# qiqiqicheng/news-recommendation-tc

Measured on AMD Instinct MI355X. Metric: recalled pairs/sec (YouTubeDNN top-30) + DIN scored pairs/sec, 1/2/4/8 MI355X, higher is better.
Workload: dtype fp16

## Files before the change

### news-recommendation-tc_amd/csrc/ip_topk.hip

```cpp
#include "nrk_common.h"

#include <float.h>
#include <math.h>
#include <stdlib.h>

#include <algorithm>
#include <type_traits>
#include <utility>

namespace nrk {

typedef float f32x16 __attribute__((ext_vector_type(16)));
typedef _Float16 f16x8 __attribute__((ext_vector_type(8)));
typedef unsigned u32x4 __attribute__((ext_vector_type(4)));
typedef float f32x4 __attribute__((ext_vector_type(4)));

constexpr int IP_KFAST = 128;
constexpr int IP_KMAX = 2048;
#ifndef NRK_SCAN_TILE
#define NRK_SCAN_TILE 8192
#endif
constexpr int SCAN_TILE = NRK_SCAN_TILE;
#ifndef NRK_SCAN_TB128
#define NRK_SCAN_TB128 4
// ... 30 lines not shown
static inline size_t catalog_body_bytes(int64_t n_items, int dp) {
    return (size_t)n_blocks_of(n_items) * 64u * (size_t)dp;
}
__host__ __device__ static inline bool catalog_has_hb(int dp) { return dp <= 64; }
__host__ __device__ static inline size_t catalog_hb_offset(int64_t n_items, int dp) {
    return (size_t)n_blocks_of(n_items) * 64u * (size_t)dp + CATALOG_HDR;
}

__global__ void catalog_pack_kernel(const float* __restrict__ items, int64_t n_items, int dim,
                                    int dp, const CatalogHdr* __restrict__ hdr,
                                    uint4* __restrict__ out) {
    const int ds = dp / 16;
    const float scale = hdr->scale;
    const int64_t total = n_blocks_of(n_items) * ds * 64;
    for (int64_t t = blockIdx.x * (int64_t)blockDim.x + threadIdx.x; t < total;
         t += (int64_t)gridDim.x * blockDim.x) {
        const int lane = (int)(t & 63);
        const int s = (int)((t >> 6) % ds);
        const int64_t b = (t >> 6) / ds;
        const int64_t item = b * 32 + (lane & 31);
        const int d0 = 16 * s + 8 * (lane >> 5);
        uint16_t v[8];
#pragma unroll
        for (int e = 0; e < 8; ++e) {
            const int d = d0 + e;
            const float f = (item < n_items && d < dim) ? items[item * dim + d] : 0.0f;
            v[e] = __builtin_bit_cast(uint16_t, (_Float16)(f * scale));
        }
        uint4 o;
        o.x = v[0] | ((uint32_t)v[1] << 16);
        o.y = v[2] | ((uint32_t)v[3] << 16);
        o.z = v[4] | ((uint32_t)v[5] << 16);
        o.w = v[6] | ((uint32_t)v[7] << 16);
        out[t] = o;
    }
}

__global__ void catalog_pack_hb_kernel(const float* __restrict__ items, int64_t n_items, int dim,
                                       int dp, const CatalogHdr* __restrict__ hdr,
                                       uint4* __restrict__ out) {
    const int ppr = dp / 8;
    const float scale = hdr->scale;
    const int64_t total = n_blocks_of(n_items) * 2 * 16 * ppr;
    for (int64_t t = blockIdx.x * (int64_t)blockDim.x + threadIdx.x; t < total;
         t += (int64_t)gridDim.x * blockDim.x) {
        const int p = (int)(t % ppr);
        const int r = (int)((t / ppr) & 15);
        const int64_t q = t / ppr / 16;
        const int64_t item = (q >> 1) * 32 + (r & 3) + 8 * (r >> 2) + 4 * (q & 1);
        uint16_t v[8];
#pragma unroll
        for (int e = 0; e < 8; ++e) {
            const int d = 8 * p + e;
            const float f = (item < n_items && d < dim) ? items[item * dim + d] : 0.0f;
            v[e] = __builtin_bit_cast(uint16_t, (_Float16)(f * scale));
        }
        out[t] = make_uint4(v[0] | ((uint32_t)v[1] << 16), v[2] | ((uint32_t)v[3] << 16),
                            v[4] | ((uint32_t)v[5] << 16), v[6] | ((uint32_t)v[7] << 16));
    }
}

__device__ __forceinline__ int cat_lanes(int dim) { return dim <= 16 ? 16 : dim <= 32 ? 32 : 64; }

__global__ void catalog_norm_kernel(const float* __restrict__ items, int64_t n_items, int dim,
                                    CatalogHdr* hdr) {
    const int lane = threadIdx.x & 63, L = cat_lanes(dim), R = WAVE / L, j = lane & (L - 1);
    const int64_t wid = (blockIdx.x * (int64_t)blockDim.x + threadIdx.x) >> 6;
    const int64_t nw = ((int64_t)gridDim.x * blockDim.x) >> 6;
    float m = 0.0f, a = 0.0f;
    for (int64_t r0 = wid * R; r0 < n_items; r0 += nw * R) {
        const int64_t r = r0 + lane / L;
        float s = 0.0f;
        if (r < n_items) {
            const float* row = items + r * dim;
            for (int d = j; d < dim; d += L) {
                const float x = row[d];
                s += x * x;
                a = fmaxf(a, fabsf(x));
            }
        }
        for (int o = L >> 1; o > 0; o >>= 1) s += __shfl_xor(s, o, WAVE);
        if (r < n_items) m = fmaxf(m, sqrtf(s));
    }
#pragma unroll
    for (int o = 32; o > 0; o >>= 1) {
        m = fmaxf(m, __shfl_xor(m, o, WAVE));
        a = fmaxf(a, __shfl_xor(a, o, WAVE));
    }
    if ((threadIdx.x & 63) == 0) {
        atomicMax((unsigned int*)&hdr->max_norm, __float_as_uint(m));
        atomicMax((unsigned int*)&hdr->max_abs, __float_as_uint(a));
    }
}

__global__ void catalog_dnorm_kernel(const float* __restrict__ items, int64_t n_items, int dim,
                                     CatalogHdr* hdr) {
    const float scale = hdr->scale;
    const int lane = threadIdx.x & 63, L = cat_lanes(dim), R = WAVE / L, j = lane & (L - 1);
    const int64_t wid = (blockIdx.x * (int64_t)blockDim.x + threadIdx.x) >> 6;
    const int64_t nw = ((int64_t)gridDim.x * blockDim.x) >> 6;
    double m = 0.0;
    for (int64_t r0 = wid * R; r0 < n_items; r0 += nw * R) {
        const int64_t r = r0 + lane / L;
        double s = 0.0;
        if (r < n_items) {
            const float* row = items + r * dim;
            for (int d = j; d < dim; d += L) {
                const float f = row[d];
                const float x = (float)(_Float16)(f * scale);
                const double e = (double)x / (double)scale - (double)f;
                s += e * e;
            }
        }
        for (int o = L >> 1; o > 0; o >>= 1) s += __shfl_xor(s, o, WAVE);
        if (r < n_items) m = fmax(m, sqrt(s));
    }
#pragma unroll
    for (int o = 32; o > 0; o >>= 1) m = fmax(m, __shfl_xor(m, o, WAVE));
    if ((threadIdx.x & 63) == 0) atomicMax((unsigned int*)&hdr->max_dnorm, __float_as_uint((float)(m * (1.0 + 1e-6))));
}

__global__ void catalog_hdr_kernel(CatalogHdr* hdr, int dim, int dp) {
    hdr->dim = dim;
    hdr->dp = dp;
    hdr->scale = pow2_scale(hdr->max_abs);
}

__device__ __forceinline__ float round_down_sub(float theta, float two_eps) {
    float c = theta - two_eps;
    return __uint_as_float(c > 0.0f ? __float_as_uint(c) - 1u
                                    : (c == 0.0f ? 0x80000001u : __float_as_uint(c) + 1u));
}

__device__ __forceinline__ uint32_t partner32(uint32_t v, int h) {
    const auto r = __builtin_amdgcn_permlane32_swap(v, v, false, false);
    return h ? (uint32_t)r[0] : (uint32_t)r[1];
}
__device__ __forceinline__ float partner32f(float v, int h) {
    return __uint_as_float(partner32(__float_as_uint(v), h));
}

__device__ __forceinline__ float pair_min32(float v) {
    const auto r = __builtin_amdgcn_permlane32_swap(__float_as_uint(v), __float_as_uint(v), false, false);
    return fminf(__uint_as_float((uint32_t)r[0]), __uint_as_float((uint32_t)r[1]));
}

__device__ __forceinline__ uint32_t add_if(uint32_t x, uint64_t m) {
    uint32_t r;
    uint64_t co;
    asm("v_addc_co_u32_e64 %0, %1, %2, 0, %3" : "=v"(r), "=s"(co) : "v"(x), "s"(m));
    (void)co;
    return r;
}

template <int MT>
__device__ __forceinline__ void top_insert(float (&t)[MT], float v) {
#pragma unroll
    for (int i = MT - 1; i >= 1; --i) t[i] = __builtin_amdgcn_fmed3f(t[i], t[i - 1], v);
    t[0] = fmaxf(t[0], v);
}

#ifndef NRK_SCAN_STAMP
#define NRK_SCAN_STAMP 0
#endif

constexpr int SCAN_PRE_MAX = 64, SCAN_PRE_MIN = 128, SCAN_PRE_DIV = 6, SCAN_SHARD_PRE_DIV = 6;
template <int F, int T>
__device__ __forceinline__ uint32_t sel_mask_c(uint64_t m) {
    uint32_t r;
    asm("v_cndmask_b32_e64 %0, %1, %2, %3" : "=v"(r) : "n"(F), "n"(T), "s"(m));
    return r;
}
template <int T>
__device__ __forceinline__ uint32_t sel_mask_v(uint64_t m, uint32_t f) {
    uint32_t r;
    asm("v_cndmask_b32_e64 %0, %1, %2, %3" : "=v"(r) : "v"(f), "n"(T), "s"(m));
    return r;
}
template <int TB>
__device__ __forceinline__ uint32_t first_set_block(const uint64_t (&am)[TB]) {
    if constexpr (TB == 1) {
        return 0u;
    } else {
        uint32_t bs = sel_mask_c<TB - 1, TB - 2>(am[TB - 2]);
        static_for<TB - 2>([&](auto bc) {
            constexpr int b = TB - 3 - decltype(bc)::value;
            bs = sel_mask_v<b>(am[b], bs);
        });
        return bs;
    }
}
#if NRK_SCAN_STAMP
__device__ unsigned long long scan_stamps[1024 * 16];
#define SC_STAMP(k)                                           \
    do {                                                      \
        const uint64_t t_now_ = __builtin_readcyclecounter(); \
        sstp[k] += t_now_ - t_prev;                           \
        t_prev = t_now_;                                      \
    } while (0)
#else
#define SC_STAMP(k) \
    do {            \
    } while (0)
#endif

template <int MT>
__device__ __forceinline__ void list_bound_out(const float (&t)[MT], bool live, int h, int user, int n_users, int jk,
                                               float* __restrict__ bnd, int bnd_m, const float4* __restrict__ uinfo) {
    const int nl = jk + 1;
    float c[2 * MT];
#pragma unroll
    for (int i = 0; i < MT; ++i) {
        c[i] = t[i];
        c[2 * MT - 1 - i] = partner32f(t[i], h);
    }
#pragma unroll
    for (int d = MT; d >= 1; d >>= 1)
#pragma unroll
        for (int i = 0; i < 2 * MT; ++i)
            if ((i & d) == 0) {
                const float x = c[i], y = c[i + d];
                c[i] = fmaxf(x, y);
                c[i + d] = fminf(x, y);
            }
    if (h == 0 && user < n_users) {
        float* o = bnd + (size_t)user * bnd_m;
        const int p0 = 2 * (MT - nl);
        const float4 ui = uinfo[user];
        const double inv = 1.0 / (double)ui.z;
#pragma unroll
        for (int j = 0; j < 2 * MT; ++j) {
            const int r = j - p0;
            if (r >= 0 && r < bnd_m) {
                float v = -INFINITY;
                if (live && c[j] != -INFINITY) {
                    const double tv = (double)c[j] * inv - (double)ui.w;
                    v = (float)tv;
                    if ((double)v > tv) v = nextafterf(v, -INFINITY);
                }
                o[r] = v;
            }
        }
        for (int r = 2 * nl; r < bnd_m; ++r) o[r] = -INFINITY;
    }
}

template <int DS>
__device__ __forceinline__ void scan_user_setup(const float* __restrict__ users, int n_users, int dim, int user,
                                                int h, float vmax, float dvmax, float sv_scale, f16x8 (&uf)[DS],
                                                float& eps, float& scl, bool& live) {
    constexpr int DP = DS * 16;
    const bool active = user < n_users;
    float uval[DS][8];
    float nrm2 = 0.0f, uabs = 0.0f;
    const float* urow = users + (size_t)(active ? user : 0) * dim;
#pragma unroll
    for (int s = 0; s < DS; ++s)
#pragma unroll
        for (int e = 0; e < 8; ++e) {
            const int d = 16 * s + 8 * h + e;
            const float f = (active && d < dim) ? urow[d] : 0.0f;
            uval[s][e] = f;
            nrm2 += f * f;
            uabs = fmaxf(uabs, fabsf(f));
        }
    nrm2 += __shfl_xor(nrm2, 32, WAVE);
    uabs = fmaxf(uabs, __shfl_xor(uabs, 32, WAVE));
    const float su = pow2_scale(uabs);
    float du2 = 0.0f;
#pragma unroll
    for (int s = 0; s < DS; ++s)
#pragma unroll
        for (int e = 0; e < 8; ++e) {
            const float a = uval[s][e] * su;
            uf[s][e] = (_Float16)a;
            const float d = (float)uf[s][e] - a;
            du2 += d * d;
        }
    du2 += __shfl_xor(du2, 32, WAVE);
    const float nu = sqrtf(nrm2), ndu = sqrtf(du2) / su;
    const float ceps = 3.0517578e-5f + (float)DP * 1.1920929e-7f;
    eps = (nrm2 == 0.0f) ? 0.0f : (ndu * vmax + nu * dvmax + ndu * dvmax + ceps * nu * vmax) * 1.0001f + 1e-30f;
    scl = su * sv_scale;
    live = active && nrm2 > 0.0f;
}

template <int DP, int NW, int NSL, int UG, int MT, int WPE>
__global__ __launch_bounds__(NW * 64, WPE) void ip_scan_kernel(
    const float* __restrict__ users, int n_users, const uint8_t* __restrict__ catalog, int n_items, int dim, int k,
    int m2, uint2* __restrict__ app, int32_t* __restrict__ acnt, float4* __restrict__ uinfo, int tile_lo,
    int tile_hi, int n_pre, int pstride, float* __restrict__ bnd, int bnd_m) {
    constexpr int DS = DP / 16;
    constexpr int BLOCK_BYTES = 64 * DP;
    constexpr int TB = scan_tb(DP);
    constexpr int TILE_BYTES = TB * BLOCK_BYTES;
    constexpr int LPT = TILE_BYTES / (NW * 1024);
    static_assert(LPT >= 1 && LPT * NW * 1024 == TILE_BYTES, "tile split");
    static_assert(NSL >= 2, "ring");
    __shared__ __attribute__((aligned(16))) uint8_t smem[NSL * TILE_BYTES];

    const int tid = threadIdx.x;
    const int wave = tid >> 6, lane = tid & 63, h = lane >> 5, q = lane & 31;
    const int ub = blockIdx.x;
    const int ubase = ub * (NW * 32 * UG) + wave * (32 * UG);
#if NRK_SCAN_STAMP
    uint64_t sstp[8] = {0, 0, 0, 0, 0, 0, 0, 0};
    uint64_t t_prev = 0;
#endif

    const int nblk = (n_items + 31) >> 5;
    const int ntile = tile_hi;
    const CatalogHdr* hdr = reinterpret_cast<const CatalogHdr*>(catalog + (size_t)nblk * BLOCK_BYTES);
    const float vmax = hdr->max_norm, sv_scale = hdr->scale, dvmax = hdr->max_dnorm;
    const int jk = (k + 1) / 2 - 1;

    f16x8 ufrag[UG][DS];
    float eps_s[UG], tau[UG];
    float t[UG][MT];
    bool live[UG];
#pragma unroll
    for (int g = 0; g < UG; ++g) {
        const int user = ubase + g * 32 + q;
        float eps, scl;
        scan_user_setup<DS>(users, n_users, dim, user, h, vmax, dvmax, sv_scale, ufrag[g], eps, scl, live[g]);
        eps_s[g] = eps * scl;
        if (h == 0 && user < n_users) uinfo[user] = make_float4(-INFINITY, eps_s[g], scl, eps);
        tau[g] = live[g] ? -FLT_MAX : INFINITY;
#pragma unroll
        for (int i = 0; i < MT; ++i) t[g][i] = (live[g] && i >= MT - 1 - jk) ? -INFINITY : INFINITY;
    }
    uint2* const wapp = app + (size_t)(ub * (NW * 32 * UG) + __builtin_amdgcn_readfirstlane(wave) * (32 * UG)) *
                                  2 * (size_t)m2;
    uint32_t pos[UG], lim[UG];
#pragma unroll
    for (int g = 0; g < UG; ++g) {
        pos[g] = (uint32_t)((g * 32 + q) * 2 + h) * (uint32_t)m2;
        lim[g] = pos[g] + (uint32_t)m2 - 1u;
    }
    auto slot = [&](uint32_t x, int g) -> uint32_t { return min(x, lim[g]); };
    auto app_store_if = [&](uint64_t m, uint32_t e, uint2 v) {
        const uint32_t off = e << 3;
        const uint64_t d = ((uint64_t)v.y << 32) | v.x;
        uint64_t sv;
// ... 417 lines not shown
            scan_user_setup<DS>(users, n_users, dim, ubase + g * 32 + q, h, vmax, dvmax, sv_scale, ufrag[g], eps, scl,
                                live);
        }
#if NRK_SCAN_WS_PRIO
        __builtin_amdgcn_s_setprio(NRK_SCAN_WS_PRIO);
#endif
        const uint32_t lds0 = lds_base + lane * 16;
        auto pf_issue = [&](int sl, int b, u32x4 (&af)[DS]) {
            const uint32_t base = lds0 + (uint32_t)(sl * TILE_BYTES + b * DS * 1024);
            asm volatile("ds_read_b128 %0, %2 offset:0\n\tds_read_b128 %1, %2 offset:1024"
                         : "=&v"(af[0]), "=&v"(af[1])
                         : "v"(base)
                         : "memory");
        };
        auto pf_wait_issue = [&](u32x4 (&cur)[DS], int sl, int b, u32x4 (&nxt)[DS]) {
            const uint32_t base = lds0 + (uint32_t)(sl * TILE_BYTES + b * DS * 1024);
            asm volatile("s_waitcnt lgkmcnt(0)\n\tds_read_b128 %0, %4 offset:0\n\tds_read_b128 %1, %4 offset:1024"
                         : "=&v"(nxt[0]), "=&v"(nxt[1]), "+v"(cur[0]), "+v"(cur[1])
                         : "v"(base)
                         : "memory");
        };
        auto pf_wait = [&](u32x4 (&cur)[DS]) {
            asm volatile("s_waitcnt lgkmcnt(0)" : "+v"(cur[0]), "+v"(cur[1])::"memory");
        };
        auto tile = [&](auto nt_c, const int (&tt)[TPS], const int (&sl)[TPS], const uint32_t (&ms)[TPS],
                        auto mask_c) __attribute__((always_inline)) {
            constexpr int NT = decltype(nt_c)::value, NBK = NT * TB;
            constexpr bool MASK = decltype(mask_c)::value;
            float mx[2][UG];
            using P5 = float[5];
            auto red1 = [&](const f32x16& a, int bb, P5& pm) __attribute__((always_inline)) {
                float x[16];
#pragma unroll
                for (int r = 0; r < 16; ++r) {
                    x[r] = a[r];
                    if constexpr (MASK) {
                        const int row = (tt[bb / TB] * TB + bb % TB) * 32 + (r & 3) + 8 * (r >> 2) + 4 * h;
                        if (row >= n_items) x[r] = -INFINITY;
                    }
                }
                auto m3 = [](float p, float s, float u) { return fmaxf(fmaxf(p, s), u); };
                pm[0] = m3(x[0], x[1], x[2]);
                pm[1] = m3(x[3], x[4], x[5]);
                pm[2] = m3(x[6], x[7], x[8]);
                pm[3] = m3(x[9], x[10], x[11]);
                pm[4] = fmaxf(m3(x[12], x[13], x[14]), x[15]);
            };
            auto red2 = [&](const P5& pm, int bb, int gg) __attribute__((always_inline)) {
                mx[bb & 1][gg] = fmaxf(fmaxf(fmaxf(fmaxf(pm[0], pm[1]), pm[2]), pm[3]), pm[4]);
            };
            auto put = [&](int bb) __attribute__((always_inline)) {
                const f32x4 v0 = {mx[bb & 1][0], mx[bb & 1][1], mx[bb & 1][2], mx[bb & 1][3]};
                const f32x4 v1 = {mx[bb & 1][4], mx[bb & 1][5], mx[bb & 1][6], mx[bb & 1][7]};
                asm volatile("ds_write_b128 %0, %1 offset:0\n\tds_write_b128 %0, %2 offset:1024" ::"v"(
                                 ms[bb / TB] + (uint32_t)((bb % TB) * 2048)),
                             "v"(v0), "v"(v1)
                             : "memory");
            };
            auto slb = [&](int bb) { return sl[bb / TB]; };
            constexpr int NSTEP = NBK * UG;
            f32x16 acc[2];
            float pm[2][5];
            u32x4 afp[DS], afb[DS];
            pf_issue(slb(0), 0, afp);
            static_for<NBK>([&](auto bc) {
                constexpr int bb = decltype(bc)::value;
                u32x4 afn[DS];
                if constexpr (bb + 1 < NBK) pf_wait_issue(afp, slb(bb + 1), (bb + 1) % TB, afn);
                else pf_wait(afp);
#pragma unroll
                for (int s = 0; s < DS; ++s) afb[s] = afp[s];
                if constexpr (bb + 1 < NBK) {
#pragma unroll
                    for (int s = 0; s < DS; ++s) afp[s] = afn[s];
                }
                static_for<UG>([&](auto gc) {
                    constexpr int g = decltype(gc)::value, j = bb * UG + g;
                    f32x16& A = acc[j & 1];
                    A = __builtin_amdgcn_mfma_f32_32x32x16_f16(__builtin_bit_cast(f16x8, afb[0]), ufrag[g][0],
                                                               f32x16{}, 0, 0, 0);
                    if constexpr (j >= 2) red2(pm[j & 1], (j - 2) / UG, (j - 2) % UG);
                    if constexpr (!MASK) {
                        __builtin_amdgcn_sched_group_barrier(0x008, 1, 0);
                        if constexpr (j >= 2) __builtin_amdgcn_sched_group_barrier(0x002, 3, 0);
                    }
                    A = __builtin_amdgcn_mfma_f32_32x32x16_f16(__builtin_bit_cast(f16x8, afb[1]), ufrag[g][1], A, 0,
                                                               0, 0);
                    if constexpr (j >= 1) red1(acc[(j - 1) & 1], (j - 1) / UG, pm[(j - 1) & 1]);
                    if constexpr (bb > 0 && g == 2) put(bb - 1);
                    if constexpr (!MASK) {
                        __builtin_amdgcn_sched_group_barrier(0x008, 1, 0);
                        if constexpr (j >= 1) __builtin_amdgcn_sched_group_barrier(0x002, 6, 0);
                        __builtin_amdgcn_sched_barrier(0);
                    }
                });
            });
            red2(pm[(NSTEP - 2) & 1], (NSTEP - 2) / UG, (NSTEP - 2) % UG);
            red1(acc[(NSTEP - 1) & 1], (NSTEP - 1) / UG, pm[(NSTEP - 1) & 1]);
            red2(pm[(NSTEP - 1) & 1], (NSTEP - 1) / UG, (NSTEP - 1) % UG);
            put(NBK - 1);
        };
#pragma unroll
        for (int p = 0; p < DAHEAD; ++p) issue_step(p);
        for (int p = 0; p <= NP; ++p) {
            SC_STAMP(7);
            sync();
            SC_STAMP(0);
            issue_step(p + DAHEAD);
            int tts[TPS], sls[TPS];
            uint32_t mss[TPS];
#pragma unroll
            for (int t = 0; t < TPS; ++t) {
                const int i = min(TPS * p + t, nseq - 1);
                tts[t] = seq(i);
                sls[t] = (TPS * p + t) % NSL;
                mss[t] = mx_base + (uint32_t)(((p & 1) * TPS + t) * MXS);
            }
            if (TPS * p + TPS <= nseq) {
                bool full = true;
#pragma unroll
                for (int t = 0; t < TPS; ++t) full = full && tts[t] < full_tiles;
                if (full) tile(std::integral_constant<int, TPS>{}, tts, sls, mss, std::false_type{});
                else tile(std::integral_constant<int, TPS>{}, tts, sls, mss, std::true_type{});
            } else if (TPS * p < nseq) {
                tile(std::integral_constant<int, 1>{}, tts, sls, mss, std::true_type{});
            }
            SC_STAMP(1);
        }
        asm volatile("s_waitcnt vmcnt(0)" ::: "memory");
#if NRK_SCAN_STAMP
        SC_STAMP(2);
        stamp_out();
#endif
        return;
    }

    const int gb = ((wv - NPW) / NPW) * UGB;
    float eps_s[UGB], tau[UGB];
    float t[UGB][MT];
    bool live[UGB];
#pragma unroll
    for (int g = 0; g < UGB; ++g) {
        f16x8 uf[DS];
        float eps, scl;
        const int user = ubase + (gb + g) * 32 + q;
        scan_user_setup<DS>(users, n_users, dim, user, h, vmax, dvmax, sv_scale, uf, eps, scl, live[g]);
        eps_s[g] = eps * scl;
        if (h == 0 && user < n_users) uinfo[user] = make_float4(-INFINITY, eps_s[g], scl, eps);
        tau[g] = live[g] ? -FLT_MAX : INFINITY;
#pragma unroll
        for (int i = 0; i < MT; ++i) t[g][i] = (live[g] && i >= MT - 1 - jk) ? -INFINITY : INFINITY;
    }
    uint2* const wapp = app + (size_t)(ubase + gb * 32) * 2 * (size_t)m2;
    const uint32_t pos0 = (uint32_t)(q * 2 + h) * (uint32_t)m2;
    const uint32_t gstride = 64u * (uint32_t)m2;
    uint32_t pos[UGB];
#pragma unroll
    for (int g = 0; g < UGB; ++g) pos[g] = pos0 + (uint32_t)g * gstride;
    auto slot = [&](uint32_t x, int g) { return min(x, pos0 + (uint32_t)g * gstride + (uint32_t)m2 - 1u); };
    auto app_store_if = [&](uint64_t m, uint32_t e, uint2 v) {
        const uint32_t off = e << 3;
        const uint64_t d = ((uint64_t)v.y << 32) | v.x;
        uint64_t sv;
        asm volatile(
            "s_and_saveexec_b64 %0, %1\n\t"
            "global_store_dwordx2 %2, %3, %4\n\t"
            "s_mov_b64 exec, %0"
            : "=&s"(sv)
            : "s"(m), "v"(off), "v"(d), "s"(wapp)
            : "memory", "scc");
    };
    auto retau = [&](int g) {
        const float lb = pair_min32(t[g][MT - 1]);
        const float c = lb - 2.0f * eps_s[g];
        const float tv = fmaxf(__builtin_fmaf(fabsf(c), -0x1p-22f, c) - 0x1p-120f, -FLT_MAX);
        tau[g] = live[g] ? tv : INFINITY;
    };
    int next_s = n_pre > 0 ? tile_lo : INT_MAX, left_s = n_pre;
#if NRK_SCAN_STAMP
    t_prev = __builtin_readcyclecounter();
#endif
    const uint32_t mq = mx_base + (uint32_t)(gb / 4) * 1024u;
    f32x4 rr[TPS][TB][UGB / 4];
    auto read_issue = [&](int t, uint32_t a) {
        if constexpr (NB == 2) {
            asm volatile(
                "ds_read_b128 %0, %4 offset:0\n\tds_read_b128 %1, %4 offset:2048\n\t"
                "ds_read_b128 %2, %4 offset:4096\n\tds_read_b128 %3, %4 offset:6144"
                : "=&v"(rr[t][0][0]), "=&v"(rr[t][1][0]), "=&v"(rr[t][2][0]), "=&v"(rr[t][3][0])
                : "v"(a)
                : "memory");
        } else {
            asm volatile(
                "ds_read_b128 %0, %8 offset:0\n\tds_read_b128 %1, %8 offset:1024\n\t"
                "ds_read_b128 %2, %8 offset:2048\n\tds_read_b128 %3, %8 offset:3072\n\t"
                "ds_read_b128 %4, %8 offset:4096\n\tds_read_b128 %5, %8 offset:5120\n\t"
                "ds_read_b128 %6, %8 offset:6144\n\tds_read_b128 %7, %8 offset:7168"
                : "=&v"(rr[t][0][0]), "=&v"(rr[t][0][1]), "=&v"(rr[t][1][0]), "=&v"(rr[t][1][1]),
                  "=&v"(rr[t][2][0]), "=&v"(rr[t][2][1]), "=&v"(rr[t][3][0]), "=&v"(rr[t][3][1])
                : "v"(a)
                : "memory");
        }
    };
    static_assert(TPS <= 2, "read_wait");
    auto read_wait = [&](int t, bool left) {
        constexpr int L1 = TB * (UGB / 4);
        if constexpr (NB == 2) {
            if (left)
                asm volatile("s_waitcnt lgkmcnt(%4)"
                             : "+v"(rr[t][0][0]), "+v"(rr[t][1][0]), "+v"(rr[t][2][0]), "+v"(rr[t][3][0])
                             : "n"(L1)
                             : "memory");
            else
                asm volatile("s_waitcnt lgkmcnt(0)"
                             : "+v"(rr[t][0][0]), "+v"(rr[t][1][0]), "+v"(rr[t][2][0]), "+v"(rr[t][3][0])::"memory");
        } else {
            if (left)
                asm volatile("s_waitcnt lgkmcnt(%8)"
                             : "+v"(rr[t][0][0]), "+v"(rr[t][0][1]), "+v"(rr[t][1][0]), "+v"(rr[t][1][1]),
                               "+v"(rr[t][2][0]), "+v"(rr[t][2][1]), "+v"(rr[t][3][0]), "+v"(rr[t][3][1])
                             : "n"(L1)
                             : "memory");
            else
                asm volatile("s_waitcnt lgkmcnt(0)"
                             : "+v"(rr[t][0][0]), "+v"(rr[t][0][1]), "+v"(rr[t][1][0]), "+v"(rr[t][1][1]),
                               "+v"(rr[t][2][0]), "+v"(rr[t][2][1]), "+v"(rr[t][3][0]), "+v"(rr[t][3][1])::"memory");
        }
    };
    float vtp[UGB];
#pragma unroll
    for (int g = 0; g < UGB; ++g) vtp[g] = -INFINITY;
    for (int p = 0; p <= NP; ++p) {
        SC_STAMP(5);
        sync();
        SC_STAMP(0);
        if (p == 0) continue;
        const int p1 = p - 1;
#pragma unroll
        for (int t = 0; t < TPS; ++t)
            if (TPS * p1 + t < nseq) read_issue(t, mq + (uint32_t)(((p1 & 1) * TPS + t) * MXS));
        static_for<TPS>([&](auto tc) {
        constexpr int T = decltype(tc)::value;
        const int j = TPS * p1 + T;
        if (j >= nseq) return;
        read_wait(T, T + 1 < TPS && j + 1 < nseq);
        const int tt = seq(j);
        const bool pre = j < n_pre;
        if (j == n_pre) {
#pragma unroll
            for (int g = 0; g < UGB; ++g) retau(g);
        }
        bool ins_ok = true;
        if (!pre && tt == next_s) {
            ins_ok = false;
            next_s = --left_s > 0 ? next_s + pstride : INT_MAX;
        }
        const auto& r = rr[T];
        SC_STAMP(1);
#if NRK_SCAN_WS_FLOOR
        if (r[0][0][0] != 12345.0f) return;
#endif
        const uint32_t hb0 = (uint32_t)(tt * TB * 2) + (uint32_t)h;
        static_for<UGB>([&](auto gc) {
            constexpr int g = decltype(gc)::value;
            float mx[TB];
#pragma unroll
            for (int b = 0; b < TB; ++b) mx[b] = r[b][g / 4][g % 4];
            const float vt = fmaxf(fmaxf(mx[0], mx[1]), fmaxf(mx[2], mx[3]));
            if (!pre) {
                uint64_t am[TB], gm = 0, multi = 0;
#pragma unroll
                for (int b = 0; b < TB; ++b) {
                    am[b] = __builtin_amdgcn_ballot_w64(mx[b] >= tau[g]);
                    multi |= gm & am[b];
                    gm |= am[b];
                }
                if (gm) {
                    const uint32_t fid = (first_set_block<TB>(am) << 1) + hb0;
                    const uint32_t p0 = pos[g];
                    app_store_if(gm, slot(p0, g), make_uint2(__float_as_uint(vt), fid));
                    uint32_t p = add_if(p0, gm);
                    if (multi) {
                        p = p0;
#pragma unroll
                        for (int b = 0; b < TB; ++b) {
                            app_store_if(am[b] & multi, slot(p, g), make_uint2(__float_as_uint(mx[b]), hb0 + 2u * b));
                            p = add_if(p, am[b]);
                        }
                    }
                    pos[g] = p;
                }
            }
            SC_STAMP(2);
            if (pre) {
                const bool in = vt > t[g][MT - 1];
                if (__builtin_amdgcn_ballot_w64(in)) top_insert<MT>(t[g], in ? vt : -INFINITY);
            } else {
                const float vi = fmaxf(ins_ok ? vt : -INFINITY, vtp[g]);
                if (T + 1 < TPS || ((j - n_pre) & (insp - 1)) < insp - TPS) {
                    vtp[g] = vi;
                } else {
                    vtp[g] = -INFINITY;
                    const bool in = vi > t[g][MT - 1];
                    if (__builtin_amdgcn_ballot_w64(in)) {
                        top_insert<MT>(t[g], in ? vi : -INFINITY);
                        if (!pre) retau(g);
                    }
                }
            }
            SC_STAMP(4);
        });
        });
    }
    {
#pragma unroll
        for (int g = 0; g < UGB; ++g) {
            const bool in = vtp[g] > t[g][MT - 1];
            top_insert<MT>(t[g], in ? vtp[g] : -INFINITY);
        }
    }
    asm volatile("s_waitcnt vmcnt(0)" ::: "memory");
#if NRK_SCAN_STAMP
    SC_STAMP(3);
    stamp_out();
#endif
#pragma unroll
    for (int g = 0; g < UGB; ++g) {
        const float lb = pair_min32(t[g][MT - 1]);
        const int user = ubase + (gb + g) * 32 + q;
        if (user < n_users) {
            acnt[(size_t)user * 2 + h] = (int)(pos[g] - (pos0 + (uint32_t)g * gstride));
            if (h == 0) reinterpret_cast<float*>(uinfo + user)[0] = live[g] ? lb : -INFINITY;
        }
    }
    if constexpr (MT <= 32) {
        if (bnd != nullptr) {
#pragma unroll
            for (int g = 0; g < UGB; ++g)
                list_bound_out<MT>(t[g], live[g], h, ubase + (gb + g) * 32 + q, n_users, jk, bnd, bnd_m, uinfo);
        }
    }
}

__device__ __forceinline__ uint32_t fkey(float f) {
    const uint32_t b = __float_as_uint(f);
    return (b >> 31) ? ~b : (b | 0x80000000u);
}
__device__ __forceinline__ float fkey_inv(uint32_t k) {
    return __uint_as_float((k >> 31) ? (k & 0x7FFFFFFFu) : ~k);
}

template <int E>
__device__ __forceinline__ void lds_ranks(const uint32_t* __restrict__ row, int c, const uint32_t (&mine)[E],
                                          int pos, int (&rank)[E]) {
#pragma unroll
    for (int e = 0; e < E; ++e) rank[e] = 0;
    for (int j0 = 0; j0 < c; j0 += 4) {
        const uint4 q = *reinterpret_cast<const uint4*>(row + j0);
        const uint32_t qq[4] = {q.x, q.y, q.z, q.w};
#pragma unroll
        for (int t = 0; t < 4; ++t) {
#pragma unroll
            for (int e = 0; e < E; ++e)
                rank[e] += (qq[t] > mine[e] || (qq[t] == mine[e] && j0 + t < e * WAVE + pos)) ? 1 : 0;
        }
    }
}

__device__ __forceinline__ uint32_t wave_sort_desc_u32(uint32_t x, int lane) {
    static_for<6>([&](auto klc) {
        constexpr int kl = decltype(klc)::value + 1, k = 1 << kl;
        static_for<kl>([&](auto jc) {
            constexpr int j = 1 << (kl - 1 - decltype(jc)::value);
            const uint32_t y = lane_xor<j>(x);
            const bool up = (lane & k) == 0;
            const bool lower = (lane & j) == 0;
            x = (lower == up) ? max(x, y) : min(x, y);
        });
    });
    return x;
}

__device__ __forceinline__ uint32_t lds_select(uint32_t* __restrict__ row, int c, int r, int lane) {
    if (c <= WAVE) {
        wave_sync_lds();
        const uint32_t srt = wave_sort_desc_u32(lane < c ? row[lane] : 0u, lane);
        return (uint32_t)__builtin_amdgcn_readlane((int)srt, r);
    }
    if (lane < 4) row[c + lane] = 0u;
    wave_sync_lds();
    uint32_t x = 0u;
    for (int b0 = 0; b0 < c; b0 += WAVE) {
        const uint32_t mine[1] = {b0 + lane < c ? row[b0 + lane] : 0u};
        int rank[1];
        lds_ranks<1>(row, c, mine, b0 + lane, rank);
        const unsigned long long b = __ballot(b0 + lane < c && rank[0] == r);
        if (b) {
            x = (uint32_t)__shfl((int)mine[0], __ffsll((long long)b) - 1, WAVE);
            break;
        }
    }
    return x;
}

#ifndef NRK_SH_WG
#define NRK_SH_WG 6
#endif
constexpr int SH_WG_PER_CU = NRK_SH_WG;
constexpr int SH_ENT = 4;

__device__ __forceinline__ void sh_load(const uint2* s0, const uint2* s1, int a0, int n, int b0, int lane,
                                        uint2 (&ent)[SH_ENT]) {
#pragma unroll
    for (int j = 0; j < SH_ENT; ++j) {
        const int e = b0 + j * WAVE + lane;
        ent[j] = e < n ? (e < a0 ? s0[e] : s1[e - a0]) : make_uint2(0u, 0u);
    }
}

__global__ __launch_bounds__(256) void ip_select_kernel(
    int64_t n_users, int k, int m2, int bandcap, const uint2* __restrict__ app,
    const int32_t* __restrict__ acnt, const float4* __restrict__ uinfo, uint2* __restrict__ cand,
    int32_t* __restrict__ cand_cnt, float2* __restrict__ ucut, int32_t* __restrict__ ovf_flag,
    int32_t* __restrict__ ovf_list, int32_t* __restrict__ ovf_count) {
    __shared__ __attribute__((aligned(16))) uint32_t sel[4][IP_SEL + 4];
    const int lane = threadIdx.x & 63, wave = threadIdx.x >> 6;
    const int64_t nw = (int64_t)gridDim.x * 4;
    const unsigned long long lt = (1ull << lane) - 1ull;
    int64_t u = (int64_t)blockIdx.x * 4 + wave;
    int2 ac_n = make_int2(0, 0);
    float4 inf_n = make_float4(0.f, 0.f, 0.f, 0.f);
    if (u < n_users) {
        ac_n = reinterpret_cast<const int2*>(acnt)[u];
        inf_n = uinfo[u];
    }
    for (; u < n_users; u += nw) {
        const int a0 = ac_n.x, a1 = ac_n.y;
        const float4 inf = inf_n;
        if (u + nw < n_users) {
            ac_n = reinterpret_cast<const int2*>(acnt)[u + nw];
            inf_n = uinfo[u + nw];
        }
        bool ovf = a0 > m2 || a1 > m2;
        const int n = ovf ? 0 : a0 + a1;
        const uint2* s0 = app + (size_t)(2 * u) * m2;
        const uint2* s1 = s0 + m2;
        auto sh_load = [&](int n_, int b0, int lane_, uint2 (&ent)[SH_ENT]) {
#pragma unroll
            for (int j = 0; j < SH_ENT; ++j) {
                const int e = b0 + j * WAVE + lane_;
                const uint2* src = e < a0 ? s0 + e : s1 + (e - a0);
                ent[j] = e < n_ ? *src : make_uint2(0u, 0u);
            }
        };
        int c = 0;
        uint2 ent[SH_ENT];
        for (int b0 = 0; b0 < n; b0 += SH_ENT * WAVE) {
            sh_load(n, b0, lane, ent);
#pragma unroll
            for (int j = 0; j < SH_ENT; ++j) {
                const int e = b0 + j * WAVE + lane;
                const float v = __uint_as_float(ent[j].x);
                const bool kp = e < n && v >= inf.x;
                const unsigned long long bal = __ballot(kp);
                const int pos = c + __popcll(bal & lt);
                if (kp && pos < IP_SEL) sel[wave][pos] = fkey(v);
                c += __popcll(bal);
            }
        }
        if (c > IP_SEL) ovf = true;
        float theta = -INFINITY;
        wave_sync_lds();
        if (!ovf && c >= k) {
            const uint32_t x = lds_select(sel[wave], c, k - 1, lane);
            theta = fkey_inv(x);
        }
        wave_sync_lds();
        float cut = theta;
        if (inf.y != 0.0f && theta != -INFINITY) cut = round_down_sub(theta, 2.0f * inf.y);
        int nb = 0;
        uint2* bd = cand + (size_t)u * bandcap;
        for (int b0 = 0; b0 < n; b0 += SH_ENT * WAVE) {
            if (n > SH_ENT * WAVE) sh_load(n, b0, lane, ent);
#pragma unroll
// ... 1503 lines not shown
```

Before: 1.189 billion.

## Split scan loop into prefix and main phases with per-step multi-tile append

```diff
diff --git a/news-recommendation-tc_amd/csrc/ip_topk.hip b/news-recommendation-tc_amd/csrc/ip_topk.hip
--- a/news-recommendation-tc_amd/csrc/ip_topk.hip
+++ b/news-recommendation-tc_amd/csrc/ip_topk.hip
@@ -206,6 +206,17 @@
     (void)co;
     return r;
 }
+__device__ __forceinline__ void add_if_to(uint32_t& x, uint64_t m) {
+    uint64_t co;
+    asm("v_addc_co_u32_e64 %0, %1, %0, 0, %2" : "+v"(x), "=s"(co) : "s"(m));
+    (void)co;
+}
+
+__device__ __forceinline__ void sub_if_to(uint32_t& x, uint64_t m) {
+    uint64_t co;
+    asm("v_subb_co_u32_e64 %0, %1, %0, 0, %2" : "+v"(x), "=s"(co) : "s"(m));
+    (void)co;
+}
 
 template <int MT>
 __device__ __forceinline__ void top_insert(float (&t)[MT], float v) {
@@ -243,6 +254,19 @@
         });
         return bs;
     }
+}
+__device__ __forceinline__ uint32_t first_set_block8(const uint64_t (&am)[8]) {
+    uint32_t bs;
+    asm("v_cndmask_b32_e64 %0, 7, 6, %7\n\t"
+        "v_cndmask_b32_e64 %0, %0, 5, %6\n\t"
+        "v_cndmask_b32_e64 %0, %0, 4, %5\n\t"
+        "v_cndmask_b32_e64 %0, %0, 3, %4\n\t"
+        "v_cndmask_b32_e64 %0, %0, 2, %3\n\t"
+        "v_cndmask_b32_e64 %0, %0, 1, %2\n\t"
+        "v_cndmask_b32_e64 %0, %0, 0, %1"
+        : "=&v"(bs)
+        : "s"(am[0]), "s"(am[1]), "s"(am[2]), "s"(am[3]), "s"(am[4]), "s"(am[5]), "s"(am[6]));
+    return bs;
 }
 #if NRK_SCAN_STAMP
 __device__ unsigned long long scan_stamps[1024 * 16];
@@ -966,14 +990,13 @@
         for (int i = 0; i < MT; ++i) t[g][i] = (live[g] && i >= MT - 1 - jk) ? -INFINITY : INFINITY;
     }
     uint2* const wapp = app + (size_t)(ubase + gb * 32) * 2 * (size_t)m2;
-    const uint32_t pos0 = (uint32_t)(q * 2 + h) * (uint32_t)m2;
-    const uint32_t gstride = 64u * (uint32_t)m2;
-    uint32_t pos[UGB];
-#pragma unroll
-    for (int g = 0; g < UGB; ++g) pos[g] = pos0 + (uint32_t)g * gstride;
-    auto slot = [&](uint32_t x, int g) { return min(x, pos0 + (uint32_t)g * gstride + (uint32_t)m2 - 1u); };
-    auto app_store_if = [&](uint64_t m, uint32_t e, uint2 v) {
-        const uint32_t off = e << 3;
+    const uint32_t off0 = ((uint32_t)(q * 2 + h) * (uint32_t)m2) << 3;
+    const size_t gstride = 64u * (size_t)m2;
+    uint32_t cnt[UGB];
+#pragma unroll
+    for (int g = 0; g < UGB; ++g) cnt[g] = 0u;
+    auto app_store_if = [&](uint64_t m, int g, uint32_t e, uint2 v) {
+        const uint32_t off = (min(e, (uint32_t)m2 - 1u) << 3) + off0;
         const uint64_t d = ((uint64_t)v.y << 32) | v.x;
         uint64_t sv;
         asm volatile(
@@ -981,7 +1004,7 @@
             "global_store_dwordx2 %2, %3, %4\n\t"
             "s_mov_b64 exec, %0"
             : "=&s"(sv)
-            : "s"(m), "v"(off), "v"(d), "s"(wapp)
+            : "s"(m), "v"(off), "v"(d), "s"(wapp + (size_t)g * gstride)
             : "memory", "scc");
     };
     auto retau = [&](int g) {
@@ -1016,115 +1039,193 @@
                 : "memory");
         }
     };
-    static_assert(TPS <= 2, "read_wait");
-    auto read_wait = [&](int t, bool left) {
-        constexpr int L1 = TB * (UGB / 4);
+    auto read_wait = [&](int t, auto left_c) __attribute__((always_inline)) {
+        constexpr int LEFT = decltype(left_c)::value;
+        auto& r = rr[t];
         if constexpr (NB == 2) {
-            if (left)
-                asm volatile("s_waitcnt lgkmcnt(%4)"
-                             : "+v"(rr[t][0][0]), "+v"(rr[t][1][0]), "+v"(rr[t][2][0]), "+v"(rr[t][3][0])
-                             : "n"(L1)
-                             : "memory");
-            else
-                asm volatile("s_waitcnt lgkmcnt(0)"
-                             : "+v"(rr[t][0][0]), "+v"(rr[t][1][0]), "+v"(rr[t][2][0]), "+v"(rr[t][3][0])::"memory");
+            asm volatile("s_waitcnt lgkmcnt(%4)"
+                         : "+v"(r[0][0]), "+v"(r[1][0]), "+v"(r[2][0]), "+v"(r[3][0])
+                         : "n"(LEFT)
+                         : "memory");
         } else {
-            if (left)
-                asm volatile("s_waitcnt lgkmcnt(%8)"
-                             : "+v"(rr[t][0][0]), "+v"(rr[t][0][1]), "+v"(rr[t][1][0]), "+v"(rr[t][1][1]),
-                               "+v"(rr[t][2][0]), "+v"(rr[t][2][1]), "+v"(rr[t][3][0]), "+v"(rr[t][3][1])
-                             : "n"(L1)
-                             : "memory");
-            else
-                asm volatile("s_waitcnt lgkmcnt(0)"
-                             : "+v"(rr[t][0][0]), "+v"(rr[t][0][1]), "+v"(rr[t][1][0]), "+v"(rr[t][1][1]),
-                               "+v"(rr[t][2][0]), "+v"(rr[t][2][1]), "+v"(rr[t][3][0]), "+v"(rr[t][3][1])::"memory");
-        }
-    };
+            asm volatile("s_waitcnt lgkmcnt(%8)"
+                         : "+v"(r[0][0]), "+v"(r[0][1]), "+v"(r[1][0]), "+v"(r[1][1]), "+v"(r[2][0]), "+v"(r[2][1]),
+                           "+v"(r[3][0]), "+v"(r[3][1])
+                         : "n"(LEFT)
+                         : "memory");
+        }
+    };
+    auto append = [&](auto gc, const auto& mx, float vmx, uint32_t hb) __attribute__((always_inline)) {
+        constexpr int g = decltype(gc)::value;
+        constexpr int NBK = (int)std::extent_v<std::remove_reference_t<decltype(mx)>>;
+        uint64_t am[NBK], gm = 0, multi = 0;
+#pragma unroll
+        for (int b = 0; b < NBK; ++b) {
+            am[b] = __builtin_amdgcn_ballot_w64(mx[b] >= tau[g]);
+            multi |= gm & am[b];
+            gm |= am[b];
+        }
+        if (gm) {
+            uint32_t bs;
+            if constexpr (NBK == 8) bs = first_set_block8(am);
+            else bs = first_set_block<NBK>(am);
+            app_store_if(gm, g, cnt[g], make_uint2(__float_as_uint(vmx), (bs << 1) + hb));
+            add_if_to(cnt[g], gm);
+            if (__builtin_expect(multi != 0, 0)) {
+                sub_if_to(cnt[g], multi);
+                static_for<NBK / TB>([&](auto tc) {
+                    constexpr int B0 = decltype(tc)::value * TB;
+                    uint64_t at[TB], gt = 0, mt = 0;
+#pragma unroll
+                    for (int b = 0; b < TB; ++b) {
+                        at[b] = am[B0 + b] & multi;
+                        mt |= gt & at[b];
+                        gt |= at[b];
+                    }
+                    if (gt) {
+                        const float vt = fmaxf(fmaxf(mx[B0], mx[B0 + 1]), fmaxf(mx[B0 + 2], mx[B0 + 3]));
+                        const uint32_t ft = (first_set_block<TB>(at) << 1) + hb + 2u * B0;
+                        app_store_if(gt, g, cnt[g], make_uint2(__float_as_uint(vt), ft));
+                        add_if_to(cnt[g], gt);
+                        if (mt) {
+                            sub_if_to(cnt[g], mt);
+#pragma unroll
+                            for (int b = 0; b < TB; ++b) {
+                                app_store_if(at[b] & mt, g, cnt[g],
+                                             make_uint2(__float_as_uint(mx[B0 + b]), hb + 2u * (B0 + b)));
+                                add_if_to(cnt[g], at[b] & mt);
+                            }
+                        }
+                    }
+                });
+            }
+        }
+    };
+    auto step_reads = [&](int p1) {
+#pragma unroll
+        for (int t = 0; t < TPS; ++t) read_issue(t, mq + (uint32_t)(((p1 & 1) * TPS + t) * MXS));
+    };
+    auto pre_tile = [&](auto tc) __attribute__((always_inline)) {
+        constexpr int T = decltype(tc)::value;
+#pragma unroll
+        for (int g = 0; g < UGB; ++g) {
+            const auto& r = rr[T];
+            const float vt = fmaxf(fmaxf(r[0][g / 4][g % 4], r[1][g / 4][g % 4]),
+                                   fmaxf(r[2][g / 4][g % 4], r[3][g / 4][g % 4]));
+            const bool in = vt > t[g][MT - 1];
+            if (__builtin_amdgcn_ballot_w64(in)) top_insert<MT>(t[g], in ? vt : -INFINITY);
+        }
+    };
+    constexpr int L1 = TB * (UGB / 4);
     float vtp[UGB];
 #pragma unroll
     for (int g = 0; g < UGB; ++g) vtp[g] = -INFINITY;
-    for (int p = 0; p <= NP; ++p) {
+    SC_STAMP(5);
+    sync();
+    SC_STAMP(0);
+    const int PA = n_pre / TPS;
+    for (int p1 = 0; p1 < PA; ++p1) {
         SC_STAMP(5);
         sync();
         SC_STAMP(0);
-        if (p == 0) continue;
-        const int p1 = p - 1;
-#pragma unroll
-        for (int t = 0; t < TPS; ++t)
-            if (TPS * p1 + t < nseq) read_issue(t, mq + (uint32_t)(((p1 & 1) * TPS + t) * MXS));
+        step_reads(p1);
+#if NRK_SCAN_WS_FLOOR
+        read_wait(TPS - 1, std::integral_constant<int, 0>{});
+        if (rr[TPS - 1][0][0][0] != 12345.0f) continue;
+#endif
         static_for<TPS>([&](auto tc) {
-        constexpr int T = decltype(tc)::value;
-        const int j = TPS * p1 + T;
-        if (j >= nseq) return;
-        read_wait(T, T + 1 < TPS && j + 1 < nseq);
-        const int tt = seq(j);
-        const bool pre = j < n_pre;
-        if (j == n_pre) {
-#pragma unroll
-            for (int g = 0; g < UGB; ++g) retau(g);
-        }
-        bool ins_ok = true;
-        if (!pre && tt == next_s) {
-            ins_ok = false;
-            next_s = --left_s > 0 ? next_s + pstride : INT_MAX;
-        }
-        const auto& r = rr[T];
+            constexpr int T = decltype(tc)::value;
+            read_wait(T, std::integral_constant<int, (TPS - 1 - T) * L1>{});
+            SC_STAMP(1);
+            pre_tile(tc);
+            SC_STAMP(4);
+        });
+    }
+    for (int p1 = PA; p1 < NP; ++p1) {
+        SC_STAMP(5);
+        sync();
+        SC_STAMP(0);
+        step_reads(p1);
+        const int j0 = TPS * p1;
+        static_for<TPS>([&](auto tc) { read_wait(decltype(tc)::value, std::integral_constant<int, 0>{}); });
         SC_STAMP(1);
 #if NRK_SCAN_WS_FLOOR
-        if (r[0][0][0] != 12345.0f) return;
+        if (rr[TPS - 1][0][0][0] != 12345.0f) continue;
 #endif
-        const uint32_t hb0 = (uint32_t)(tt * TB * 2) + (uint32_t)h;
+        if (p1 == PA) {
+            static_for<TPS>([&](auto tc) {
+                constexpr int T = decltype(tc)::value;
+                if (j0 + T < n_pre) {
+                    pre_tile(tc);
+#pragma unroll
+                    for (int b = 0; b < TB; ++b)
+#pragma unroll
+                        for (int c = 0; c < UGB / 4; ++c)
+                            rr[T][b][c] = f32x4{-INFINITY, -INFINITY, -INFINITY, -INFINITY};
+                }
+            });
+#pragma unroll
+            for (int g = 0; g < UGB; ++g) retau(g);
+        }
+        const bool whole = j0 + TPS <= nseq;
+        if (!whole) {
+            static_for<TPS>([&](auto tc) {
+                constexpr int T = decltype(tc)::value;
+                if (j0 + T >= nseq) {
+#pragma unroll
+                    for (int b = 0; b < TB; ++b)
+#pragma unroll
+                        for (int c = 0; c < UGB / 4; ++c)
+                            rr[T][b][c] = f32x4{-INFINITY, -INFINITY, -INFINITY, -INFINITY};
+                }
+            });
+        }
+        const int tt0 = seq(j0 + TPS - 1) - (TPS - 1);
+        bool smp[TPS], any_smp = false;
+#pragma unroll
+        for (int t = 0; t < TPS; ++t) {
+            smp[t] = tt0 + t == next_s;
+            if (smp[t]) {
+                any_smp = true;
+                next_s = --left_s > 0 ? next_s + pstride : INT_MAX;
+            }
+        }
+        uint32_t hb0 = (uint32_t)(tt0 * TB * 2) + (uint32_t)h;
+        asm volatile("" : "+v"(hb0));
         static_for<UGB>([&](auto gc) {
             constexpr int g = decltype(gc)::value;
-            float mx[TB];
-#pragma unroll
-            for (int b = 0; b < TB; ++b) mx[b] = r[b][g / 4][g % 4];
-            const float vt = fmaxf(fmaxf(mx[0], mx[1]), fmaxf(mx[2], mx[3]));
-            if (!pre) {
-                uint64_t am[TB], gm = 0, multi = 0;
-#pragma unroll
-                for (int b = 0; b < TB; ++b) {
-                    am[b] = __builtin_amdgcn_ballot_w64(mx[b] >= tau[g]);
-                    multi |= gm & am[b];
-                    gm |= am[b];
+            constexpr int NBK = TPS * TB;
+            float mx[NBK];
+#pragma unroll
+            for (int b = 0; b < NBK; ++b) mx[b] = rr[b / TB][b % TB][g / 4][g % 4];
+            float v = mx[0];
+#pragma unroll
+            for (int b = 1; b + 1 < NBK; b += 2) v = fmaxf(fmaxf(v, mx[b]), mx[b + 1]);
+            if constexpr (NBK % 2 == 0) v = fmaxf(v, mx[NBK - 1]);
+            append(gc, mx, v, hb0);
+            SC_STAMP(2);
+            float vins = v;
+            if (__builtin_expect(any_smp, 0)) {
+                vins = -INFINITY;
+#pragma unroll
+                for (int b = 0; b < NBK; ++b)
+                    if (!smp[b / TB]) vins = fmaxf(vins, mx[b]);
+            }
+            vtp[g] = fmaxf(vins, vtp[g]);
+        });
+        if (whole && ((j0 + TPS - 1 - n_pre) & (insp - 1)) >= insp - TPS) {
+#pragma unroll
+            for (int g = 0; g < UGB; ++g) {
+                const float vi = vtp[g];
+                vtp[g] = -INFINITY;
+                const bool in = vi > t[g][MT - 1];
+                if (__builtin_amdgcn_ballot_w64(in)) {
+                    top_insert<MT>(t[g], in ? vi : -INFINITY);
+                    retau(g);
                 }
-                if (gm) {
-                    const uint32_t fid = (first_set_block<TB>(am) << 1) + hb0;
-                    const uint32_t p0 = pos[g];
-                    app_store_if(gm, slot(p0, g), make_uint2(__float_as_uint(vt), fid));
-                    uint32_t p = add_if(p0, gm);
-                    if (multi) {
-                        p = p0;
-#pragma unroll
-                        for (int b = 0; b < TB; ++b) {
-                            app_store_if(am[b] & multi, slot(p, g), make_uint2(__float_as_uint(mx[b]), hb0 + 2u * b));
-                            p = add_if(p, am[b]);
-                        }
-                    }
-                    pos[g] = p;
-                }
-            }
-            SC_STAMP(2);
-            if (pre) {
-                const bool in = vt > t[g][MT - 1];
-                if (__builtin_amdgcn_ballot_w64(in)) top_insert<MT>(t[g], in ? vt : -INFINITY);
-            } else {
-                const float vi = fmaxf(ins_ok ? vt : -INFINITY, vtp[g]);
-                if (T + 1 < TPS || ((j - n_pre) & (insp - 1)) < insp - TPS) {
-                    vtp[g] = vi;
-                } else {
-                    vtp[g] = -INFINITY;
-                    const bool in = vi > t[g][MT - 1];
-                    if (__builtin_amdgcn_ballot_w64(in)) {
-                        top_insert<MT>(t[g], in ? vi : -INFINITY);
-                        if (!pre) retau(g);
-                    }
-                }
-            }
-            SC_STAMP(4);
-        });
-        });
+            }
+        }
+        SC_STAMP(4);
     }
     {
 #pragma unroll
@@ -1143,7 +1244,7 @@
         const float lb = pair_min32(t[g][MT - 1]);
         const int user = ubase + (gb + g) * 32 + q;
         if (user < n_users) {
-            acnt[(size_t)user * 2 + h] = (int)(pos[g] - (pos0 + (uint32_t)g * gstride));
+            acnt[(size_t)user * 2 + h] = (int)cnt[g];
             if (h == 0) reinterpret_cast<float*>(uinfo + user)[0] = live[g] ? lb : -INFINITY;
         }
     }
```

Measured after the change: 1.215 billion (median of 6 runs). 2.3% higher.
